# tk1363704/CAREL-VAE

Measured on AMD Instinct MI355X. Metric: clause-pairs/sec (training step), higher is better.
Workload: dtype bf16

## Files before the change

### carel_vae_amd/csrc/carel_hip_internal.h

```cpp
#pragma once
#include <hip/hip_runtime.h>
#include <stdarg.h>
#include <stdio.h>
#include "../../include/carel_hip.h"
#include "carel_common.h"

#ifdef CAREL_EXPERIMENTS
#define CAREL_TUNABLE(type, name, value) static type name = value
#else
#define CAREL_TUNABLE(type, name, value) static constexpr type name = value
#endif

namespace carel {

int set_error(int code, const char* fmt, ...);
int check_launch(const char* what);
int slab_reduce_multi(const void* slabs, void* out, int64_t n, const void* slabs2, void* out2, int64_t n2, int splits, const void* partials,
                      int nparts, void* dgamma, void* dbeta, void* dbias, hipStream_t stream);
#ifdef CAREL_EXPERIMENTS
int gemm_rowln_wanted(long rows);
int gemm_rowln_wanted_k(int K);
#else
inline int gemm_rowln_wanted(long) { return 0; }
inline int gemm_rowln_wanted_k(int) { return 0; }
#endif
void encoder_ln_resid_enable(int on);
void encoder_ln_slab_fusion_enable(int on);
void encoder_wgrad_group_enable(int on);
void adam_grid_cap(long cap);
void tail_overlap_enable(int on);
int gemm_pp_init_device(int device);
int gather_rows(const void* in_f32, const void* in_bf16, const void* idx, int n, void* out_f32, void* out_bf16, hipStream_t stream);
int scatter_rows(const void* in_f32, const void* in_bf16, const void* idx, int n, void* out_f32, void* out_bf16, hipStream_t stream);

int layernorm_bwd_rows(const void* dy, const void* h, const void* stats, const void* gamma, int64_t rows, uint32_t drop_seed, uint32_t drop_site,
                       uint32_t drop_idx_offset, float drop_p, const void* drop_row_map, void* dh_f32, void* dy_bf16, void* partials,
                       hipStream_t stream);
int layernorm_bwd_reduce(const void* partials, int64_t rows, void* dgamma, void* dbeta, void* dbias, hipStream_t stream);
int layernorm_bwd_blocks_max(int64_t rows);
int layernorm_bwd_rows_slabs(const void* slabs, int splits, const void* resid, const void* h, const void* stats, const void* gamma, int64_t rows,
                             uint32_t drop_seed, uint32_t drop_site, uint32_t drop_idx_offset, float drop_p, const void* drop_row_map, void* dh_f32,
                             void* dy_bf16, void* partials, hipStream_t stream);
int layernorm_fwd_slabs(const void* slabs, int splits, const void* bias, const void* resid, const void* resid_stats, const void* resid_gamma,
                        const void* resid_beta, uint32_t drop_seed, uint32_t drop_site, uint32_t drop_idx_offset, float drop_p, const void* drop_row_map,
                        void* h_out, const void* gamma, const void* beta, float eps, int64_t rows, void* x_f32, void* x_bf16, void* stats,
                        hipStream_t stream);

constexpr int GEMM_EX_FIXED_ROWS = 0x100;
constexpr int GEMM_EX_DEFER_EPILOGUE = 0x200;
int gemm_bf16_ex(const carel_gemm_args* a, int split_tile_factor, void* stream);
int gemm_bf16_split_plan(const carel_gemm_args* a, int split_tile_factor);
int gemm_wgrad_splits_max(int M, int N, long T);
int embed_ln_bwd_ex(const carel_embed_args* a, const void* dx0, void* dword, void* dpos, void* dtype_, void* dgamma, void* dbeta,
                    void* partials, void* row_scratch, hipStream_t stream, const void* sort_ws = nullptr);
int embed_sort_supported(const carel_embed_args* a);
size_t embed_sort_bytes();
int embed_ln_fwd_keys(const carel_embed_args* a, void* sort_ws, hipStream_t stream);
int embed_sort_rows(const carel_embed_args* a, void* sort_ws, hipStream_t stream);

struct WgradGroupProb { const void* dY; const void* X; void* dW; void* db; int M, N; };
struct WgradGroupLn { const void* partials; int nparts; void* dgamma; void* dbeta; void* dbias; };
size_t gemm_pp_wgrad_group_ws_bytes(const WgradGroupProb* pb, int n, long T);
int gemm_pp_wgrad_group_ok(const WgradGroupProb* pb, int n, long T);
int gemm_pp_wgrad_group(const WgradGroupProb* pb, int n, long T, void* ws, size_t ws_bytes, const WgradGroupLn* ln, int n_ln, hipStream_t stream);

inline Dropout make_dropout(uint32_t seed, uint32_t site, float p, uint32_t idx_offset) {
  Dropout d;
  d.key = mix32(seed + site * 0x9E3779B9u);
  d.idx_offset = idx_offset;
  if (p <= 0.f) { d.thresh = 0u; d.scale = 1.f; }
  else if (p >= 1.f) { d.thresh = 0xFFFFFFFFu; d.scale = 0.f; }
  else {
    d.thresh = (uint32_t)((double)p * 4294967296.0);
    d.scale = (float)(1.0 / (1.0 - (double)p));
    if (d.thresh == 0u) d.scale = 1.f;
  }
  return d;
}

struct AttnParams;
int attn_long_fwd(const AttnParams& q, hipStream_t stream);
int attn_long_bwd(const AttnParams& q, void* workspace, int64_t workspace_bytes, hipStream_t stream);

}
```

### carel_vae_amd/csrc/gemm.hip

```cpp
#include "gemm_epilogue.h"
#include "reduce_device.h"

namespace carel {

template <int EPI>
__global__ __launch_bounds__(256) void slab_epilogue_kernel(GemmParams p, const float* __restrict__ slabs, int splits) {
  const long chunk = (long)blockIdx.x * 256 + threadIdx.x;
  const int cpr = p.N >> 3;
  if (chunk >= (long)p.M * cpr) return;
  const long row = chunk / cpr, col = (chunk - row * cpr) * 8;
  const long off = row * p.N + col, plane = (long)p.M * p.N;
  float v[8];
  {
    const float4 a = *(const float4*)(slabs + off), b = *(const float4*)(slabs + off + 4);
    v[0] = a.x; v[1] = a.y; v[2] = a.z; v[3] = a.w; v[4] = b.x; v[5] = b.y; v[6] = b.z; v[7] = b.w;
  }
  for (int z = 1; z < splits; ++z) {
    const float4 a = *(const float4*)(slabs + z * plane + off), b = *(const float4*)(slabs + z * plane + off + 4);
    v[0] += a.x; v[1] += a.y; v[2] += a.z; v[3] += a.w; v[4] += b.x; v[5] += b.y; v[6] += b.z; v[7] += b.w;
  }
  epi_store8<EPI>(p, v, row, col);
}

template <bool AT, bool BT, int EPI, int DBG = 0>
// ... 672 lines not shown
    std::vector<float> c2;
    for (size_t i = 0; i + 1 < g_prof.cal2.size(); i += 2) {
      float t = 0.f;
      if (hipEventSynchronize(g_prof.cal2[i + 1]) == hipSuccess && hipEventElapsedTime(&t, g_prof.cal2[i], g_prof.cal2[i + 1]) == hipSuccess) c2.push_back(t);
    }
    if (!c2.empty()) { std::sort(c2.begin(), c2.end()); g_prof.last_pair_us = c2[c2.size() / 2] * 1e3; }
  }
  for (size_t i = 0; i + 1 < g_prof.used; i += 2) {
    if (hipEventSynchronize(g_prof.ev[i + 1]) != hipSuccess) return set_error(CAREL_ERR_HIP, "carel_profile_gemm_read: event sync failed");
    float t = 0.f;
    if (hipEventElapsedTime(&t, g_prof.ev[i], g_prof.ev[i + 1]) != hipSuccess) return set_error(CAREL_ERR_HIP, "carel_profile_gemm_read: elapsed failed");
    ms += (t > overhead ? t - overhead : 0.0); fl += g_prof.flops[i / 2];
  }
  *total_ms = ms; *total_flops = fl; *launches = (int64_t)(g_prof.used / 2);
  g_prof.used = 0; g_prof.flops.clear();
  return CAREL_OK;
}

extern "C" int carel_profile_gemm_overheads(double* empty_kernel_bracket_us, double* event_pair_us) {
  if (!empty_kernel_bracket_us || !event_pair_us) return set_error(CAREL_ERR_ARG, "carel_profile_gemm_overheads: null output");
  *empty_kernel_bracket_us = g_prof.last_empty_us; *event_pair_us = g_prof.last_pair_us;
  return CAREL_OK;
}

static int gemm_shape_ok(int M, int N, int K, int splits, int form) {
  if (M <= 0 || N <= 0 || K <= 0 || splits <= 0) return 0;
  if (form == CAREL_GEMM_TN) {
    if (M % 256 == 0 && N % 96 == 0 && K % 64 == 0 && (K >> 6) / splits >= 4) return 1;
  }
  const bool pp = form != CAREL_GEMM_TN && N % 96 == 0 && K >= 256;
  if (!((M % 128 == 0 && N % 128 == 0) || (M % 256 == 0 && N % 192 == 0) || pp)) return 0;
  if (K % (64 * splits)) return 0;
  return 1;
}

#ifdef CAREL_EXPERIMENTS
CAREL_TUNABLE(int, g_rowln_mode, 0);
CAREL_TUNABLE(long, g_rowln_min_rows, 6144);
namespace carel {
int gemm_rowln_wanted(long rows) { return g_rowln_mode != 0 && rows >= g_rowln_min_rows; }
int gemm_rowln_wanted_k(int K) { return g_rowln_mode == 1 || K <= 768; }
}
extern "C" int carel_gemm_rowln(const carel_gemm_rowln_args* a, void* stream_) {
  hipStream_t stream = (hipStream_t)stream_;
  if (!a) return set_error(CAREL_ERR_ARG, "carel_gemm_rowln: null args");
  if (a->M < 1 || a->K < 128 || (a->K & 127)) return set_error(CAREL_ERR_SHAPE, "carel_gemm_rowln: M >= 1 and K a multiple of 128 (M=%d K=%d)", a->M, a->K);
  if (!a->A || !a->W || !a->resid_f32 || !a->gamma || !a->beta) return set_error(CAREL_ERR_ARG, "carel_gemm_rowln: null operand");
  if ((((uintptr_t)a->A | (uintptr_t)a->W | (uintptr_t)a->resid_f32 | (uintptr_t)a->gamma | (uintptr_t)a->beta | (uintptr_t)a->bias | (uintptr_t)a->h_f32 |
        (uintptr_t)a->x_f32 | (uintptr_t)a->x_bf16) & 15) || (a->lda & 7) || a->lda < a->K || (!a->w_packed && ((a->ldb & 7) || a->ldb < a->K)))
    return set_error(CAREL_ERR_ARG, "carel_gemm_rowln: operands must be 16-byte aligned, leading dimensions multiples of 8 and >= K");
  RowLnParams p;
  p.A = (const bf16_t*)a->A; p.lda = a->lda; p.W = (const bf16_t*)a->W; p.ldb = a->ldb; p.bias = (const float*)a->bias; p.resid = (const float*)a->resid_f32;
  p.gamma = (const float*)a->gamma; p.beta = (const float*)a->beta; p.eps = a->eps;
  p.h_out = (float*)a->h_f32; p.x_f32 = (float*)a->x_f32; p.x_bf16 = (bf16_t*)a->x_bf16; p.stats = (float*)a->stats; p.M = a->M; p.K = a->K;
  p.drop = make_dropout(a->drop_seed, a->drop_site, a->drop_p, a->drop_idx_offset); p.drop_row_map = (const int*)a->drop_row_map;
  ProfScope prof_scope(stream, 2.0 * (double)a->M * 768.0 * (double)a->K);
  return gemm_rowln_launch(p, a->w_packed != 0, stream);
}
extern "C" int carel_gemm_rowln_pack(const void* W, int64_t ldb, int32_t K, void* out, void* stream) {
  if (!W || !out || K < 128 || (K & 127) || ldb < K || (ldb & 7) || (((uintptr_t)W | (uintptr_t)out) & 15))
    return set_error(CAREL_ERR_ARG, "carel_gemm_rowln_pack: bad arguments (K multiple of 128, ldb >= K multiple of 8, 16-byte aligned pointers)");
  return gemm_rowln_pack(W, (long)ldb, K, out, (hipStream_t)stream);
}

extern "C" int carel_gemm_set_variant(int32_t v) {
  if (v >= 20 && v <= 23) { g_xcd_n = 1 << (v - 20); return CAREL_OK; }
  if (v == 24) { g_xcd_n = 0; return CAREL_OK; }
  if (v == 30 || v == 31) { g_big_auto = v - 30; return CAREL_OK; }
  if (v >= 50 && v <= 59) { g_pp_min_tiles = (v - 50) * 32; return CAREL_OK; }
  if (v >= 340 && v <= 342) { g_sm_mode = v - 340; return CAREL_OK; }
  if (v >= 330 && v <= 333) { g_resid_split = v - 330; return CAREL_OK; }
  if (v >= 40 && v <= 49) { g_pp_min_tiles_k768 = (v - 40) * 32; return CAREL_OK; }
  if (v >= 70 && v <= 73) { gemm_pp_force_npn(v - 70); return CAREL_OK; }
  if (v >= 100 && v <= 116) { gemm_pp_wgrad_force(v - 100); return CAREL_OK; }
  if (v == 130 || v == 131) { g_auto_split_min_k = v == 130 ? 1536 : 768; return CAREL_OK; }
  if (v == 140 || v == 141) { g_pp_split = v - 140; return CAREL_OK; }
  if (v == 160 || v == 161) { gemm_pp_gelu_lut(v - 160); return CAREL_OK; }
  if (v >= 190 && v <= 192) { g_rowln_mode = v - 190; return CAREL_OK; }
  if (v >= 193 && v <= 195) { gemm_rowln_dbg(v - 193); return CAREL_OK; }
  if (v == 270 || v == 271) { encoder_ln_slab_fusion_enable(v - 270); return CAREL_OK; }
  if (v >= 250 && v <= 252) { gemm_pp_group_mode(v - 250); return CAREL_OK; }
  if (v == 240 || v == 241) { encoder_wgrad_group_enable(v - 240); return CAREL_OK; }
  if (v == 230 || v == 231) { encoder_ln_resid_enable(v - 230); return CAREL_OK; }
  if (v >= 220 && v <= 225) { gemm_tri_enable(v - 220); return CAREL_OK; }
  if (v >= 280 && v <= 292) { adam_grid_cap(32L << (v - 280)); return CAREL_OK; }
  if (v == 210 || v == 211) { tail_overlap_enable(v - 210); return CAREL_OK; }
  if (v == 200 || v == 201) { gemm_pp_pair_enable(v - 200); return CAREL_OK; }
  if (v == 170 || v == 171) { gemm_pp_epi_prefetch(v - 170); return CAREL_OK; }
  if (v == 120 || v == 121) { gemm_pp_xcd_rect(v - 120); return CAREL_OK; }
  if (v == 90 || v == 91) { gemm_pp_wide_variant(v - 90); return CAREL_OK; }
  g_gemm_variant = v;
  return CAREL_OK;
}
#endif

static int gemm_prepare(const carel_gemm_args* a, int split_tile_factor, PlannedGemm* out) {
  if (!a) return set_error(CAREL_ERR_ARG, "carel_gemm_bf16: null args");
  const int splits = a->splits > 0 ? a->splits : 1;
  if (!gemm_shape_ok(a->M, a->N, a->K, splits, a->form))
    return set_error(CAREL_ERR_SHAPE, "carel_gemm_bf16: (M,N) must be multiples of (128,128) or (256,192) and K of 64*splits (M=%d N=%d K=%d splits=%d)",
                     a->M, a->N, a->K, splits);
  if (!a->A || !a->B) return set_error(CAREL_ERR_ARG, "carel_gemm_bf16: null operand");
  if (((uintptr_t)a->A | (uintptr_t)a->B) & 15 || (a->lda & 7) || (a->ldb & 7) || (a->ldc & 3))
    return set_error(CAREL_ERR_ARG, "carel_gemm_bf16: operands must be 16-byte aligned, ld multiples of 8");
  GemmParams p = {};
  p.A = (const bf16_t*)a->A; p.B = (const bf16_t*)a->B; p.lda = a->lda; p.ldb = a->ldb;
  p.M = a->M; p.N = a->N; p.K = a->K / splits;
  p.out0 = (bf16_t*)a->out_bf16; p.out1 = (bf16_t*)a->out2_bf16; p.outf = (float*)a->out_f32; p.ldc = a->ldc;
  p.bias = (const float*)a->bias; p.resid = (const float*)a->resid_f32; p.aux = (const bf16_t*)a->aux_bf16;
  p.resid_stats = (const float*)a->resid_ln_stats; p.resid_gamma = (const float*)a->resid_ln_gamma; p.resid_beta = (const float*)a->resid_ln_beta;
  if (p.resid_stats || p.resid_gamma || p.resid_beta) {
    if (a->epilogue != EPI_BIAS_DROP_RESID || !p.resid_stats || !p.resid_gamma || !p.resid_beta)
      return set_error(CAREL_ERR_ARG, "carel_gemm_bf16: resid_ln_stats / _gamma / _beta go together and with CAREL_EPI_BIAS_DROP_RESID only");
    if ((((uintptr_t)p.resid_stats) & 7) || (((uintptr_t)p.resid_gamma | (uintptr_t)p.resid_beta) & 15))
      return set_error(CAREL_ERR_ARG, "carel_gemm_bf16: resid_ln_* pointers must be 8 / 16-byte aligned");
  }
  p.drop = make_dropout(a->drop_seed, a->drop_site, a->drop_p, a->drop_idx_offset);
  p.tiles_m = a->M / 128; p.tiles_n = a->N / 128;
  p.split_tile_factor = split_tile_factor;
  p.xcd_n = (a->form == CAREL_GEMM_TN && g_xcd_n <= 1) ? 8 : g_xcd_n;
  p.splitk_ws = (float*)a->splitk_ws; p.splitk_ws_bytes = a->splitk_ws ? (size_t)a->splitk_ws_bytes : 0;
  p.pair_flags = nullptr; p.pair_seq = 0;
  if (a->splitk_ws && a->splitk_ws_zeroed && (size_t)a->splitk_ws_bytes > (size_t)(64 << 20) && ((uintptr_t)a->splitk_ws & 15) == 0 && (a->splitk_ws_bytes & 15) == 0) {
    p.splitk_ws_bytes -= PP_PAIR_FLAG_BYTES;
    p.pair_flags = (unsigned*)((char*)a->splitk_ws + p.splitk_ws_bytes);
  }
  if (a->ldc != a->N) p.splitk_ws = nullptr;
  if (a->colsum_part) p.splitk_ws = nullptr;
  p.colsum_part = (float*)a->colsum_part; p.drop_row_map = (const int*)a->drop_row_map; p.colsum_a = (float*)a->colsum_a;
  if (p.colsum_a && a->form != CAREL_GEMM_TN) return set_error(CAREL_ERR_ARG, "carel_gemm_bf16: colsum_a is a TN-form (wgrad) option");
  const int form = a->form, epi = a->epilogue;
  if (splits != 1 && epi != EPI_SLAB_F32) return set_error(CAREL_ERR_ARG, "carel_gemm_bf16: split-K only with the slab epilogue");
#define NEED(ptr, what) if (!(ptr)) return set_error(CAREL_ERR_ARG, "carel_gemm_bf16: epilogue needs " what)
  switch (epi) {
    case EPI_BIAS_BF16: NEED(p.out0, "out_bf16"); break;
    case EPI_BIAS_GELU: NEED(p.out1, "out2_bf16"); break;
    case EPI_BIAS_GELU_DG: NEED(p.out0, "out_bf16"); NEED(p.out1, "out2_bf16"); break;
    case EPI_BIAS_DROP_RESID: NEED(p.outf, "out_f32"); NEED(p.resid, "resid_f32"); break;
    case EPI_DGELU_BF16: case EPI_MUL_BF16: NEED(p.out0, "out_bf16"); NEED(p.aux, "aux_bf16"); break;
    case EPI_ADD_F32: NEED(p.outf, "out_f32"); break;
    case EPI_SLAB_F32: NEED(p.outf, "out_f32"); break;
    default: return set_error(CAREL_ERR_ARG, "carel_gemm_bf16: unknown epilogue %d", epi);
  }
#undef NEED
  if (epi != EPI_BIAS_DROP_RESID && epi != EPI_ADD_F32 && epi != EPI_SLAB_F32 && (a->ldc & 7))
    return set_error(CAREL_ERR_ARG, "carel_gemm_bf16: bf16 outputs and aux need ldc a multiple of 8 (ldc=%ld)", (long)a->ldc);
  const auto fn = launch_instance(form, epi);
  if (!fn) return set_error(CAREL_ERR_ARG, "carel_gemm_bf16: unsupported form/epilogue combination (%d,%d)", form, epi);
  *out = PlannedGemm{p, splits, gemm_plan(p, form, epi, splits, a->K), fn};
  if (form == CAREL_GEMM_TN && out->plan.family == PLAN_PP) out->p.K = a->K;
  if (out->plan.family == PLAN_NONE)
    return set_error(CAREL_ERR_SHAPE, "carel_gemm_bf16: no kernel of this form takes the shape (M=%d N=%d K=%d splits=%d)", a->M, a->N, a->K, splits);
  return CAREL_OK;
}

extern "C" int carel_gemm_bf16(const carel_gemm_args* a, void* stream_) { return carel::gemm_bf16_ex(a, 1, stream_); }

int carel::gemm_bf16_split_plan(const carel_gemm_args* a, int split_tile_factor) {
  PlannedGemm g;
  return gemm_prepare(a, split_tile_factor, &g) ? 1 : g.plan.slabs;
}

#ifdef CAREL_EXPERIMENTS
extern "C" int carel_gemm_split_plan(const carel_gemm_args* a, int32_t flags, int32_t* plan) {
  if (!plan) return set_error(CAREL_ERR_ARG, "carel_gemm_split_plan: null plan");
  if (flags & ~(0xff | GEMM_EX_FIXED_ROWS)) return set_error(CAREL_ERR_ARG, "carel_gemm_split_plan: flags are a chain count | CAREL_PLAN_FIXED_ROWS");
// ... 97 lines not shown
```

### carel_vae_amd/csrc/ln.hip

```cpp
#include "carel_hip_internal.h"
#include "ln_device.h"
#include "reduce_device.h"

namespace carel {

__global__ __launch_bounds__(256) void ln_fwd_kernel(const float* __restrict__ h, const float* __restrict__ gamma,
                                                     const float* __restrict__ beta, float eps, long rows,
                                                     float* __restrict__ x_f32, bf16_t* __restrict__ x_bf16,
                                                     float* __restrict__ stats) {
  const int lane = threadIdx.x & 63;
  const long row = (long)blockIdx.x * 4 + (threadIdx.x >> 6);
  if (row >= rows) return;
  Row X = load_row(h + row * H, lane);
  const Row G = load_row(gamma, lane), Bt = load_row(beta, lane);
  float mean, rstd;
  ln_normalise(X, G, Bt, eps, mean, rstd);
  if (x_f32) store_row(x_f32 + row * H, lane, X);
  if (x_bf16) store_row_bf16(x_bf16 + row * H, lane, X);
  if (stats && lane == 0) { stats[row * 2] = mean; stats[row * 2 + 1] = rstd; }
}

struct LnFwdSlabs {
  const float* slabs; int splits; long plane;
  const float* bias; const float* resid; const float* resid_stats; const float* resid_gamma; const float* resid_beta;
// ... 35 lines not shown
  float mean, rstd;
  ln_normalise(X, G, Bt, eps, mean, rstd);
  if (x_f32) store_row(x_f32 + row * H, lane, X);
  if (x_bf16) store_row_bf16(x_bf16 + row * H, lane, X);
  if (stats && lane == 0) { stats[row * 2] = mean; stats[row * 2 + 1] = rstd; }
}

struct EmbedArgs {
  const long* ids; const long* tt;
  const float* word; const float* pos; const float* type;
  const float* gamma; const float* beta;
  float eps; int S; long rows; int roberta; int pad_id; int vocab, max_pos, type_vocab;
  Dropout drop;
  const int* tok_row;
};

__device__ __forceinline__ int position_id(const EmbedArgs& a, long row, int lane) {
  const int s = (int)(row % a.S);
  if (!a.roberta) return s;
  const long base = row - s;
  int cnt = 0;
  for (int c0 = 0; c0 <= s; c0 += 64) {
    const int j = c0 + lane;
    const bool nz = (j <= s) && (a.ids[base + j] != a.pad_id);
    cnt += __popcll(__ballot(nz));
  }
  const bool self_nz = a.ids[row] != a.pad_id;
  return (self_nz ? cnt : 0) + a.pad_id;
}

__device__ __forceinline__ Row embed_gather(const EmbedArgs& a, long row, int lane, int& pid, int& tid_) {
  long id = a.ids[row];
  id = id < 0 ? 0 : (id >= a.vocab ? a.vocab - 1 : id);
  pid = position_id(a, row, lane);
  pid = pid >= a.max_pos ? a.max_pos - 1 : pid;
  long t = a.tt ? a.tt[row] : 0;
  tid_ = (int)(t < 0 ? 0 : (t >= a.type_vocab ? a.type_vocab - 1 : t));
  Row A = load_row(a.word + id * H, lane);
  const Row B = load_row(a.pos + (long)pid * H, lane), Cc = load_row(a.type + (long)tid_ * H, lane);
  ROW_FOREACH(a = a + b + c; (void)e)
  return A;
}

__global__ __launch_bounds__(256) void embed_fwd_kernel(EmbedArgs a, float* __restrict__ x_f32, bf16_t* __restrict__ x_bf16,
                                                        float* __restrict__ stats, int2* __restrict__ row_keys) {
  const int lane = threadIdx.x & 63;
  const long orow = (long)blockIdx.x * 4 + (threadIdx.x >> 6);
  if (orow >= a.rows) return;
  const long row = a.tok_row ? (long)a.tok_row[orow] : orow;
  if (row_keys && lane == 0 && row < 0) row_keys[orow] = int2{-1, -1};
  if (row < 0) {
    Row Z;
#pragma unroll
    for (int i = 0; i < NV; ++i) Z.v[i] = float4{0.f, 0.f, 0.f, 0.f};
    store_row(x_f32 + orow * H, lane, Z);
    store_row_bf16(x_bf16 + orow * H, lane, Z);
    if (lane == 0) { stats[orow * 2] = 0.f; stats[orow * 2 + 1] = 0.f; }
    return;
  }
  int pid, tid_;
  Row X = embed_gather(a, row, lane, pid, tid_);
  if (row_keys && lane == 0) {
    long id = a.ids[row];
    id = id < 0 ? 0 : (id >= a.vocab ? a.vocab - 1 : id);
    row_keys[orow] = int2{(int)id, pid};
  }
  const Row G = load_row(a.gamma, lane), Bt = load_row(a.beta, lane);
  float mean, rstd;
  ln_normalise(X, G, Bt, a.eps, mean, rstd);
  if (a.drop.thresh) {
#pragma unroll
    for (int i = 0; i < NV; ++i) {
      const uint32_t e0 = (uint32_t)(row * H + (i * 64 + lane) * 4);
      float dm[4];
      dropout_mult_n<4>(a.drop, e0, dm);
      X.v[i].x *= dm[0]; X.v[i].y *= dm[1]; X.v[i].z *= dm[2]; X.v[i].w *= dm[3];
    }
  }
  store_row(x_f32 + orow * H, lane, X);
  store_row_bf16(x_bf16 + orow * H, lane, X);
  if (lane == 0) { stats[orow * 2] = mean; stats[orow * 2 + 1] = rstd; }
}

__device__ __forceinline__ void ln_bwd_row(Row& DY , Row& XH , const Row& G,
                                           float mean, float rstd) {
  float s1 = 0.f, s2 = 0.f;
#pragma unroll
  for (int i = 0; i < NV; ++i) {
    float* d = &DY.v[i].x; float* x = &XH.v[i].x; const float* g = &G.v[i].x;
#pragma unroll
    for (int e = 0; e < 4; ++e) {
      const float xh = (x[e] - mean) * rstd;
      const float dxh = d[e] * g[e];
      s1 += dxh; s2 += dxh * xh;
      x[e] = xh;
    }
  }
  s1 = wave_sum(s1) * (1.0f / H);
  s2 = wave_sum(s2) * (1.0f / H);
#pragma unroll
  for (int i = 0; i < NV; ++i) {
    float* d = &DY.v[i].x; float* x = &XH.v[i].x; const float* g = &G.v[i].x;
#pragma unroll
    for (int e = 0; e < 4; ++e) {
      const float dy = d[e], xh = x[e];
      d[e] = rstd * (dy * g[e] - s1 - xh * s2);
      x[e] = dy * xh;
    }
  }
}

constexpr int LNB_ROWS = 16;

__device__ __forceinline__ void write_partials(float* lds , const Row& acc, float* __restrict__ dst, int lane, int wave) {
  __syncthreads();
  store_row(lds + wave * H, lane, acc);
  __syncthreads();
  for (int c = threadIdx.x; c < H; c += 256) dst[c] = (lds[c] + lds[H + c]) + (lds[2 * H + c] + lds[3 * H + c]);
}

struct LnSlabSrc { int splits; long plane; const float* resid; };
template <bool SLAB, int RPW = 4>
__global__ __launch_bounds__(256) void ln_bwd_kernel(const float* __restrict__ dy_out, const float* __restrict__ h,
                                                     const float* __restrict__ stats, const float* __restrict__ gamma,
                                                     long rows, Dropout drop, const int* __restrict__ row_map,
                                                     float* __restrict__ dh, bf16_t* __restrict__ dyb,
                                                     float* __restrict__ partials, LnSlabSrc src) {
  __shared__ float lds[4 * H];
  const int lane = threadIdx.x & 63, wave = threadIdx.x >> 6;
  const Row G = load_row(gamma, lane);
  Row accG, accB, accBias;
#pragma unroll
  for (int i = 0; i < NV; ++i) accG.v[i] = accB.v[i] = accBias.v[i] = float4{0.f, 0.f, 0.f, 0.f};
  constexpr int WG_ROWS = 4 * RPW;
  Row DYr[RPW], XHr[RPW];
  float mr[RPW], rr[RPW];
  int dr[RPW];
  const int* rm = row_map ? row_map : (const int*)stats;
#pragma unroll
  for (int k = 0; k < RPW; ++k) {
    const long row = (long)blockIdx.x * WG_ROWS + wave + 4 * k;
    const long lrow = row < rows ? row : rows - 1;
    DYr[k] = load_row(dy_out + lrow * H, lane);
    if constexpr (SLAB) {
      for (int z = 1; z < src.splits; ++z) {
        const Row Z = load_row(dy_out + (long)z * src.plane + lrow * H, lane);
#pragma unroll
        for (int i = 0; i < NV; ++i) { DYr[k].v[i].x += Z.v[i].x; DYr[k].v[i].y += Z.v[i].y; DYr[k].v[i].z += Z.v[i].z; DYr[k].v[i].w += Z.v[i].w; }
      }
      if (src.resid) {
        const Row R = load_row(src.resid + lrow * H, lane);
#pragma unroll
        for (int i = 0; i < NV; ++i) { DYr[k].v[i].x += R.v[i].x; DYr[k].v[i].y += R.v[i].y; DYr[k].v[i].z += R.v[i].z; DYr[k].v[i].w += R.v[i].w; }
      }
    }
    XHr[k] = load_row(h + lrow * H, lane);
    mr[k] = stats[lrow * 2]; rr[k] = stats[lrow * 2 + 1];
    dr[k] = rm[lrow];
  }
#pragma unroll
  for (int k = 0; k < RPW; ++k) {
    const long row = (long)blockIdx.x * WG_ROWS + wave + 4 * k;
    if (row >= rows) break;
    Row DY = DYr[k];
    Row XH = XHr[k];
    const float mean = mr[k], rstd = rr[k];
#pragma unroll
    for (int i = 0; i < NV; ++i) { accB.v[i].x += DY.v[i].x; accB.v[i].y += DY.v[i].y; accB.v[i].z += DY.v[i].z; accB.v[i].w += DY.v[i].w; }
    ln_bwd_row(DY, XH, G, mean, rstd);
#pragma unroll
    for (int i = 0; i < NV; ++i) { accG.v[i].x += XH.v[i].x; accG.v[i].y += XH.v[i].y; accG.v[i].z += XH.v[i].z; accG.v[i].w += XH.v[i].w; }
    if (dh) store_row(dh + row * H, lane, DY);
    if (drop.thresh) {
      const long drow = row_map ? (long)dr[k] : row;
#pragma unroll
      for (int i = 0; i < NV; ++i) {
        const uint32_t e0 = (uint32_t)(drow * H + (i * 64 + lane) * 4);
        float dm[4];
        dropout_mult_n<4>(drop, e0, dm);
        DY.v[i].x *= dm[0]; DY.v[i].y *= dm[1]; DY.v[i].z *= dm[2]; DY.v[i].w *= dm[3];
      }
    }
    if (dyb) store_row_bf16(dyb + row * H, lane, DY);
#pragma unroll
    for (int i = 0; i < NV; ++i) { accBias.v[i].x += DY.v[i].x; accBias.v[i].y += DY.v[i].y; accBias.v[i].z += DY.v[i].z; accBias.v[i].w += DY.v[i].w; }
  }
  float* dst = partials + (long)blockIdx.x * 3 * H;
  write_partials(lds, accG, dst, lane, wave);
  write_partials(lds, accB, dst + H, lane, wave);
  write_partials(lds, accBias, dst + 2 * H, lane, wave);
}

__global__ __launch_bounds__(256) void pos_reduce_kernel(const float* __restrict__ rows, int B, int S, float* __restrict__ dpos) {
  const long e = ((long)blockIdx.x * 256 + threadIdx.x) * 4;
  if (e >= (long)S * H) return;
  float4 acc = float4{0.f, 0.f, 0.f, 0.f};
  for (int b = 0; b < B; b += 4) {
    float4 v[4];
#pragma unroll
    for (int u = 0; u < 4; ++u) v[u] = (b + u < B) ? *(const float4*)(rows + (long)(b + u) * S * H + e) : float4{0.f, 0.f, 0.f, 0.f};
#pragma unroll
    for (int u = 0; u < 4; ++u) { acc.x += v[u].x; acc.y += v[u].y; acc.z += v[u].z; acc.w += v[u].w; }
  }
  *(float4*)(dpos + e) = acc;
}

constexpr int EMB_SORT_MAX = 8192, EMB_ROW_BITS = 13;
__global__ __launch_bounds__(1024) void embed_sort_kernel(const int2* __restrict__ row_keys, int rows, uint32_t* __restrict__ out) {
  __shared__ uint32_t k[EMB_SORT_MAX];
  const int which = (int)blockIdx.x;
  int n = 64;
  while (n < rows) n <<= 1;
  for (int i = threadIdx.x; i < n; i += 1024) {
    uint32_t key = 0xFFFFFFFFu;
    if (i < rows) {
      const int2 v = row_keys[i];
      const int id = which ? v.y : v.x;
      if (id >= 0) key = ((uint32_t)id << EMB_ROW_BITS) | (uint32_t)i;
    }
    k[i] = key;
  }
  __syncthreads();
  for (int size = 2; size <= n; size <<= 1)
    for (int stride = size >> 1; stride > 0; stride >>= 1) {
      for (int t = threadIdx.x; t < (n >> 1); t += 1024) {
        const int lo = 2 * t - (t & (stride - 1)), hi = lo + stride;
        const bool up = (lo & size) == 0;
        const uint32_t a = k[lo], b = k[hi];
        if ((a > b) == up) { k[lo] = b; k[hi] = a; }
      }
      __syncthreads();
    }
  for (int i = threadIdx.x; i < EMB_SORT_MAX; i += 1024) out[which * EMB_SORT_MAX + i] = i < n ? k[i] : 0xFFFFFFFFu;
}

__global__ __launch_bounds__(256) void embed_segsum_kernel(const uint32_t* __restrict__ keys, const float* __restrict__ rows, float* __restrict__ table,
                                                           int table_rows) {
  const int lane = threadIdx.x & 63;
  const int w = (int)blockIdx.x * 4 + (int)(threadIdx.x >> 6);
  const int pos = w / 3, chunk = w - pos * 3;
  if (pos >= EMB_SORT_MAX) return;
  const uint32_t key = keys[pos];
  if (key == 0xFFFFFFFFu) return;
  const uint32_t id = key >> EMB_ROW_BITS;
  if ((int)id >= table_rows) return;
  if (pos > 0 && (keys[pos - 1] >> EMB_ROW_BITS) == id) return;
  const float* src = rows + chunk * 256 + lane * 4;
  float4 acc = float4{0.f, 0.f, 0.f, 0.f};
  for (int base = pos; base < EMB_SORT_MAX; base += 64) {
    const uint32_t kj = base + lane < EMB_SORT_MAX ? keys[base + lane] : 0xFFFFFFFFu;
    const unsigned long long m = __ballot(kj != 0xFFFFFFFFu && (kj >> EMB_ROW_BITS) == id);
    const int cnt = m == ~0ull ? 64 : __ffsll((long long)~m) - 1;
#pragma unroll 8
    for (int t = 0; t < cnt; ++t) {
      const uint32_t r = (uint32_t)__shfl((int)kj, t, 64) & (uint32_t)(EMB_SORT_MAX - 1);
      const float4 v = *(const float4*)(src + (long)r * H);
      acc.x += v.x; acc.y += v.y; acc.z += v.z; acc.w += v.w;
    }
    if (cnt < 64) break;
  }
  *(float4*)(table + (long)id * H + chunk * 256 + lane * 4) = acc;
}

__global__ __launch_bounds__(256) void embed_bwd_kernel(EmbedArgs a, const float* __restrict__ dx0,
                                                        const float* __restrict__ stats, float* __restrict__ dword,
                                                        float* __restrict__ dpos, float* __restrict__ partials,
                                                        float* __restrict__ row_out, int word_atomic, int pos_atomic) {
  __shared__ float lds[4 * H];
  const int lane = threadIdx.x & 63, wave = threadIdx.x >> 6;
  const Row G = load_row(a.gamma, lane);
  Row accG, accB, accT0, accT1;
#pragma unroll
  for (int i = 0; i < NV; ++i) accG.v[i] = accB.v[i] = accT0.v[i] = accT1.v[i] = float4{0.f, 0.f, 0.f, 0.f};
  for (int r = wave; r < LNB_ROWS; r += 4) {
// ... 205 lines not shown
}
int embed_sort_rows(const carel_embed_args* a, void* sort_ws, hipStream_t stream) {
  const long rows = (a->tok_row && a->n_rows > 0) ? (long)a->n_rows : (long)a->batch * a->seq_len;
  hipLaunchKernelGGL(embed_sort_kernel, dim3(2), dim3(1024), 0, stream, (const int2*)sort_ws, (int)rows, (uint32_t*)((char*)sort_ws + (size_t)EMB_SORT_MAX * 8));
  return check_launch("embed_sort_kernel");
}
}

extern "C" int carel_embed_ln_bwd_blocks(int64_t rows) { return (int)((rows + LNB_ROWS - 1) / LNB_ROWS); }

namespace carel {
int embed_ln_bwd_ex(const carel_embed_args* a, const void* dx0, void* dword, void* dpos, void* dtype_, void* dgamma, void* dbeta,
                    void* partials, void* row_scratch, hipStream_t stream, const void* sort_ws) {
  int rc = embed_check(a, "carel_embed_ln_bwd");
  if (rc) return rc;
  if (!dx0 || !dword || !dpos || !dtype_ || !dgamma || !dbeta || !partials || !a->stats)
    return set_error(CAREL_ERR_ARG, "carel_embed_ln_bwd: null tensor");
  EmbedArgs e = make_embed(a);
  const int nblk = carel_embed_ln_bwd_blocks(e.rows);
  const int slots = 2 + e.type_vocab;
  const bool by_reduction = row_scratch && !e.roberta && !e.tok_row && e.rows == (long)a->batch * a->seq_len;
  const bool sorted = row_scratch && sort_ws && embed_sort_supported(a);
  hipLaunchKernelGGL(embed_bwd_kernel, dim3(nblk), dim3(256), 0, stream, e, (const float*)dx0, (const float*)a->stats,
                     (float*)dword, (float*)dpos, (float*)partials, (by_reduction || sorted) ? (float*)row_scratch : (float*)nullptr,
                     sorted ? 0 : 1, (by_reduction || sorted) ? 0 : 1);
  rc = check_launch("embed_bwd_kernel");
  if (rc) return rc;
  if (by_reduction) {
    hipLaunchKernelGGL(pos_reduce_kernel, dim3((unsigned)(((long)a->seq_len * H / 4 + 255) / 256)), dim3(256), 0, stream,
                       (const float*)row_scratch, a->batch, a->seq_len, (float*)dpos);
    if ((rc = check_launch("pos_reduce_kernel"))) return rc;
  }
  if (sorted) {
    const uint32_t* keys = (const uint32_t*)((const char*)sort_ws + (size_t)EMB_SORT_MAX * 8);
    const unsigned blocks = (unsigned)((EMB_SORT_MAX * 3 + 3) / 4);
    hipLaunchKernelGGL(embed_segsum_kernel, dim3(blocks), dim3(256), 0, stream, keys, (const float*)row_scratch, (float*)dword, a->vocab_size);
    if ((rc = check_launch("embed_segsum_kernel"))) return rc;
    if (!by_reduction) {
      hipLaunchKernelGGL(embed_segsum_kernel, dim3(blocks), dim3(256), 0, stream, keys + EMB_SORT_MAX, (const float*)row_scratch, (float*)dpos, a->max_pos);
      if ((rc = check_launch("embed_segsum_kernel"))) return rc;
    }
  }
  SegOuts so; so.p[0] = (float*)dgamma; so.p[1] = (float*)dbeta; so.p[2] = (float*)dtype_;
  so.p[3] = e.type_vocab > 1 ? (float*)dtype_ + H : nullptr;
  hipLaunchKernelGGL(partial_reduce_seg_kernel, dim3((slots * H + PR_COLS - 1) / PR_COLS), dim3(256), 0, stream, (const float*)partials,
                     so, H, slots * H, nblk);
  return check_launch("partial_reduce_seg_kernel");
}
}

extern "C" int carel_embed_ln_bwd(const carel_embed_args* a, const void* dx0, void* dword, void* dpos, void* dtype_,
                                  void* dgamma, void* dbeta, void* partials, void* stream_) {
  return embed_ln_bwd_ex(a, dx0, dword, dpos, dtype_, dgamma, dbeta, partials, nullptr, (hipStream_t)stream_, nullptr);
}

extern "C" int carel_layernorm_fwd(const void* h, const void* gamma, const void* beta, float eps, int64_t rows, int32_t hidden,
                                   void* x_f32, void* x_bf16, void* stats, void* stream_) {
  hipStream_t stream = (hipStream_t)stream_;
  if (hidden != H) return set_error(CAREL_ERR_SHAPE, "carel_layernorm_fwd: hidden must be %d", H);
  if (!h || !gamma || !beta || rows <= 0) return set_error(CAREL_ERR_ARG, "carel_layernorm_fwd: bad arguments");
  hipLaunchKernelGGL(ln_fwd_kernel, dim3((unsigned)((rows + 3) / 4)), dim3(256), 0, stream, (const float*)h, (const float*)gamma,
                     (const float*)beta, eps, (long)rows, (float*)x_f32, (bf16_t*)x_bf16, (float*)stats);
  return check_launch("ln_fwd_kernel");
}

static int ln_bwd_rpw(int64_t rows) { return rows <= 2048 ? 1 : (rows <= 4096 ? 2 : 4); }
extern "C" int carel_layernorm_bwd_blocks(int64_t rows) { const int wg = 4 * ln_bwd_rpw(rows); return (int)((rows + wg - 1) / wg); }
namespace carel {
int layernorm_bwd_blocks_max(int64_t rows) {
  if (rows <= 2048) return (int)((rows + 3) / 4);
  const int64_t big = (rows + 15) / 16;
  return (int)(big > 512 ? big : 512);
}
}

extern "C" int carel_layernorm_bwd(const void* dy, const void* h, const void* stats, const void* gamma, int64_t rows,
                                   int32_t hidden, uint32_t drop_seed, uint32_t drop_site, uint32_t drop_idx_offset,
                                   float drop_p, void* dh_f32, void* dy_bf16, void* dgamma, void* dbeta, void* dbias,
                                   void* partials, void* stream_) {
  return carel_layernorm_bwd_packed(dy, h, stats, gamma, rows, hidden, drop_seed, drop_site, drop_idx_offset, drop_p, nullptr, dh_f32,
                                    dy_bf16, dgamma, dbeta, dbias, partials, stream_);
}

namespace carel {
int layernorm_bwd_rows(const void* dy, const void* h, const void* stats, const void* gamma, int64_t rows, uint32_t drop_seed, uint32_t drop_site,
                       uint32_t drop_idx_offset, float drop_p, const void* drop_row_map, void* dh_f32, void* dy_bf16, void* partials,
                       hipStream_t stream) {
  if (!dy || !h || !stats || !gamma || !partials || rows <= 0) return set_error(CAREL_ERR_ARG, "carel_layernorm_bwd: bad arguments");
  const int nblk = carel_layernorm_bwd_blocks(rows);
  const Dropout drop = make_dropout(drop_seed, drop_site, drop_p, drop_idx_offset);
  const LnSlabSrc src{1, 0, nullptr};
#define CAREL_LNB(R) hipLaunchKernelGGL((ln_bwd_kernel<false, R>), dim3(nblk), dim3(256), 0, stream, (const float*)dy, (const float*)h, (const float*)stats, \
                     (const float*)gamma, (long)rows, drop, (const int*)drop_row_map, (float*)dh_f32, (bf16_t*)dy_bf16, (float*)partials, src)
  switch (ln_bwd_rpw(rows)) { case 1: CAREL_LNB(1); break; case 2: CAREL_LNB(2); break; default: CAREL_LNB(4); }
#undef CAREL_LNB
  return check_launch("ln_bwd_kernel");
}
int layernorm_bwd_rows_slabs(const void* slabs, int splits, const void* resid, const void* h, const void* stats, const void* gamma, int64_t rows,
                             uint32_t drop_seed, uint32_t drop_site, uint32_t drop_idx_offset, float drop_p, const void* drop_row_map, void* dh_f32,
                             void* dy_bf16, void* partials, hipStream_t stream) {
  if (!slabs || splits < 2 || !h || !stats || !gamma || !partials || rows <= 0) return set_error(CAREL_ERR_ARG, "layernorm_bwd_rows_slabs: bad arguments");
  const int nblk = carel_layernorm_bwd_blocks(rows);
  const Dropout drop = make_dropout(drop_seed, drop_site, drop_p, drop_idx_offset);
  const LnSlabSrc src{splits, (long)rows * H, (const float*)resid};
#define CAREL_LNB(R) hipLaunchKernelGGL((ln_bwd_kernel<true, R>), dim3(nblk), dim3(256), 0, stream, (const float*)slabs, (const float*)h, (const float*)stats, \
                     (const float*)gamma, (long)rows, drop, (const int*)drop_row_map, (float*)dh_f32, (bf16_t*)dy_bf16, (float*)partials, src)
  switch (ln_bwd_rpw(rows)) { case 1: CAREL_LNB(1); break; case 2: CAREL_LNB(2); break; default: CAREL_LNB(4); }
#undef CAREL_LNB
  return check_launch("ln_bwd_kernel<slabs>");
}
int layernorm_fwd_slabs(const void* slabs, int splits, const void* bias, const void* resid, const void* resid_stats, const void* resid_gamma,
                        const void* resid_beta, uint32_t drop_seed, uint32_t drop_site, uint32_t drop_idx_offset, float drop_p, const void* drop_row_map,
                        void* h_out, const void* gamma, const void* beta, float eps, int64_t rows, void* x_f32, void* x_bf16, void* stats,
                        hipStream_t stream) {
  if (!slabs || splits < 2 || !resid || !gamma || !beta || rows <= 0) return set_error(CAREL_ERR_ARG, "layernorm_fwd_slabs: bad arguments");
  if (resid_stats && (!resid_gamma || !resid_beta)) return set_error(CAREL_ERR_ARG, "layernorm_fwd_slabs: recomputed residual needs gamma and beta");
  LnFwdSlabs a;
  a.slabs = (const float*)slabs; a.splits = splits; a.plane = (long)rows * H; a.bias = (const float*)bias; a.resid = (const float*)resid;
  a.resid_stats = (const float*)resid_stats; a.resid_gamma = (const float*)resid_gamma; a.resid_beta = (const float*)resid_beta;
  a.drop = make_dropout(drop_seed, drop_site, drop_p, drop_idx_offset); a.row_map = (const int*)drop_row_map; a.h_out = (float*)h_out;
  hipLaunchKernelGGL(ln_fwd_slabs_kernel, dim3((unsigned)((rows + 3) / 4)), dim3(256), 0, stream, a, (const float*)gamma, (const float*)beta, eps, (long)rows,
                     (float*)x_f32, (bf16_t*)x_bf16, (float*)stats);
  return check_launch("ln_fwd_slabs_kernel");
}
int layernorm_bwd_reduce(const void* partials, int64_t rows, void* dgamma, void* dbeta, void* dbias, hipStream_t stream) {
  const int nblk = carel_layernorm_bwd_blocks(rows);
  SegOuts so; so.p[0] = (float*)dgamma; so.p[1] = (float*)dbeta; so.p[2] = (float*)dbias; so.p[3] = nullptr;
  hipLaunchKernelGGL(partial_reduce_seg_kernel, dim3((3 * H + PR_COLS - 1) / PR_COLS), dim3(256), 0, stream, (const float*)partials, so,
                     H, 3 * H, nblk);
  return check_launch("partial_reduce_seg_kernel");
}
}

extern "C" int carel_layernorm_bwd_packed(const void* dy, const void* h, const void* stats, const void* gamma, int64_t rows,
                                          int32_t hidden, uint32_t drop_seed, uint32_t drop_site, uint32_t drop_idx_offset,
                                          float drop_p, const void* drop_row_map, void* dh_f32, void* dy_bf16, void* dgamma,
                                          void* dbeta, void* dbias, void* partials, void* stream_) {
  hipStream_t stream = (hipStream_t)stream_;
  if (hidden != H) return set_error(CAREL_ERR_SHAPE, "carel_layernorm_bwd: hidden must be %d", H);
  int rc = layernorm_bwd_rows(dy, h, stats, gamma, rows, drop_seed, drop_site, drop_idx_offset, drop_p, drop_row_map, dh_f32, dy_bf16,
                              partials, stream);
  if (rc) return rc;
  return layernorm_bwd_reduce(partials, rows, dgamma, dbeta, dbias, stream);
}

extern "C" int carel_colsum_bf16(const void* x, int64_t ld, int64_t rows, int32_t n, void* out_f32, int32_t accumulate,
                                 void* partials, void* stream_) {
  hipStream_t stream = (hipStream_t)stream_;
  if (!x || !out_f32 || !partials || rows <= 0 || n <= 0 || (n & 7) || (ld & 7))
    return set_error(CAREL_ERR_ARG, "carel_colsum_bf16: bad arguments (n, ld multiples of 8)");
  const int chunks = (int)((rows + 255) / 256);
  hipLaunchKernelGGL(colsum_bf16_kernel, dim3((n + 255) / 256, chunks), dim3(256), 0, stream, (const bf16_t*)x, (long)ld,
                     (long)rows, n, (float*)partials);
  int rc = check_launch("colsum_bf16_kernel");
  if (rc) return rc;
  hipLaunchKernelGGL(partial_reduce_kernel, dim3((n + PR_COLS - 1) / PR_COLS), dim3(256), 0, stream, (const float*)partials, (float*)out_f32, n,
                     chunks, accumulate);
  return check_launch("partial_reduce_kernel");
}

extern "C" int carel_partial_reduce_f32(const void* partials, void* out, int32_t n, int32_t nparts, int32_t accumulate, void* stream_) {
  hipStream_t stream = (hipStream_t)stream_;
  if (!partials || !out || n <= 0 || nparts <= 0) return set_error(CAREL_ERR_ARG, "carel_partial_reduce_f32: bad arguments");
  hipLaunchKernelGGL(partial_reduce_kernel, dim3((n + PR_COLS - 1) / PR_COLS), dim3(256), 0, stream, (const float*)partials, (float*)out, n, nparts, accumulate);
  return check_launch("partial_reduce_kernel");
}
```

Baseline: 8423.

## Software-pipeline LayerNorm backward rows with capped VGPRs for higher occupancy

Replaces the RPW=4 LayerNorm backward kernel with a paired form. It loads one row ahead instead of holding all four rows in registers, and pins VGPRs and waves-per-EU to 4 waves. It also keeps gamma in LDS, uses a DPP/swizzle wave reduction, shrinks LDS to two rows, and uses a staged tree reduction for the partials. The aim is to raise occupancy and overlap memory latency with compute in the LN backward pass, at the cost of more barriers and possible register spills.

New measurement: 8413. No clear change (-0.1%).

```diff
diff --git a/carel_vae_amd/csrc/carel_hip_internal.h b/carel_vae_amd/csrc/carel_hip_internal.h
--- a/carel_vae_amd/csrc/carel_hip_internal.h
+++ b/carel_vae_amd/csrc/carel_hip_internal.h
@@ -27,6 +27,7 @@
 void encoder_ln_resid_enable(int on);
 void encoder_ln_slab_fusion_enable(int on);
 void encoder_wgrad_group_enable(int on);
+void ln_bwd_paired_enable(int on);
 void adam_grid_cap(long cap);
 void tail_overlap_enable(int on);
 int gemm_pp_init_device(int device);
diff --git a/carel_vae_amd/csrc/gemm.hip b/carel_vae_amd/csrc/gemm.hip
--- a/carel_vae_amd/csrc/gemm.hip
+++ b/carel_vae_amd/csrc/gemm.hip
@@ -778,6 +778,7 @@
   if (v >= 250 && v <= 252) { gemm_pp_group_mode(v - 250); return CAREL_OK; }
   if (v == 240 || v == 241) { encoder_wgrad_group_enable(v - 240); return CAREL_OK; }
   if (v == 230 || v == 231) { encoder_ln_resid_enable(v - 230); return CAREL_OK; }
+  if (v == 350 || v == 351) { ln_bwd_paired_enable(v - 350); return CAREL_OK; }
   if (v >= 220 && v <= 225) { gemm_tri_enable(v - 220); return CAREL_OK; }
   if (v >= 280 && v <= 292) { adam_grid_cap(32L << (v - 280)); return CAREL_OK; }
   if (v == 210 || v == 211) { tail_overlap_enable(v - 210); return CAREL_OK; }
diff --git a/carel_vae_amd/csrc/ln.hip b/carel_vae_amd/csrc/ln.hip
--- a/carel_vae_amd/csrc/ln.hip
+++ b/carel_vae_amd/csrc/ln.hip
@@ -141,6 +141,16 @@
   if (lane == 0) { stats[orow * 2] = mean; stats[orow * 2 + 1] = rstd; }
 }
 
+__device__ __forceinline__ float wave_sum_swz(float v) {
+  v += __int_as_float(__builtin_amdgcn_ds_bpermute((int)(((threadIdx.x & 63) ^ 32) << 2), __float_as_int(v)));
+  v += __int_as_float(__builtin_amdgcn_ds_swizzle(__float_as_int(v), (16 << 10) | 0x1f));
+  v += __int_as_float(__builtin_amdgcn_ds_swizzle(__float_as_int(v), (8 << 10) | 0x1f));
+  v += __int_as_float(__builtin_amdgcn_ds_swizzle(__float_as_int(v), (4 << 10) | 0x1f));
+  v += __int_as_float(__builtin_amdgcn_ds_swizzle(__float_as_int(v), (2 << 10) | 0x1f));
+  v += __int_as_float(__builtin_amdgcn_ds_swizzle(__float_as_int(v), (1 << 10) | 0x1f));
+  return v;
+}
+template <bool SWZ = false>
 __device__ __forceinline__ void ln_bwd_row(Row& DY , Row& XH , const Row& G,
                                            float mean, float rstd) {
   float s1 = 0.f, s2 = 0.f;
@@ -155,8 +165,8 @@
       x[e] = xh;
     }
   }
-  s1 = wave_sum(s1) * (1.0f / H);
-  s2 = wave_sum(s2) * (1.0f / H);
+  s1 = (SWZ ? wave_sum_swz(s1) : wave_sum(s1)) * (1.0f / H);
+  s2 = (SWZ ? wave_sum_swz(s2) : wave_sum(s2)) * (1.0f / H);
 #pragma unroll
   for (int i = 0; i < NV; ++i) {
     float* d = &DY.v[i].x; float* x = &XH.v[i].x; const float* g = &G.v[i].x;
@@ -178,14 +188,67 @@
   for (int c = threadIdx.x; c < H; c += 256) dst[c] = (lds[c] + lds[H + c]) + (lds[2 * H + c] + lds[3 * H + c]);
 }
 
+__device__ __forceinline__ void write_partials_staged(float* lds , const Row& acc, float* __restrict__ dst, int lane, int wave) {
+  __syncthreads();
+  if (wave & 1) store_row(lds + (wave >> 1) * H, lane, acc);
+  __syncthreads();
+  Row s = acc;
+  if (!(wave & 1)) {
+    const Row o = load_row(lds + (wave >> 1) * H, lane);
+#pragma unroll
+    for (int i = 0; i < NV; ++i) { s.v[i].x += o.v[i].x; s.v[i].y += o.v[i].y; s.v[i].z += o.v[i].z; s.v[i].w += o.v[i].w; }
+  }
+  __syncthreads();
+  if (wave == 2) store_row(lds + H, lane, s);
+  __syncthreads();
+  if (wave == 0) {
+    const Row o = load_row(lds + H, lane);
+#pragma unroll
+    for (int i = 0; i < NV; ++i) { s.v[i].x += o.v[i].x; s.v[i].y += o.v[i].y; s.v[i].z += o.v[i].z; s.v[i].w += o.v[i].w; }
+    store_row(dst, lane, s);
+  }
+}
+
 struct LnSlabSrc { int splits; long plane; const float* resid; };
-template <bool SLAB, int RPW = 4>
-__global__ __launch_bounds__(256) void ln_bwd_kernel(const float* __restrict__ dy_out, const float* __restrict__ h,
-                                                     const float* __restrict__ stats, const float* __restrict__ gamma,
-                                                     long rows, Dropout drop, const int* __restrict__ row_map,
-                                                     float* __restrict__ dh, bf16_t* __restrict__ dyb,
-                                                     float* __restrict__ partials, LnSlabSrc src) {
-  __shared__ float lds[4 * H];
+template <bool SLAB>
+__device__ __forceinline__ Row ln_bwd_load_dy(const float* __restrict__ dy_out, long lrow, int lane, const LnSlabSrc& src) {
+  Row D = load_row(dy_out + lrow * H, lane);
+  if constexpr (SLAB) {
+    for (int z = 1; z < src.splits; ++z) {
+      const Row Z = load_row(dy_out + (long)z * src.plane + lrow * H, lane);
+#pragma unroll
+      for (int i = 0; i < NV; ++i) { D.v[i].x += Z.v[i].x; D.v[i].y += Z.v[i].y; D.v[i].z += Z.v[i].z; D.v[i].w += Z.v[i].w; }
+    }
+    if (src.resid) {
+      const Row R = load_row(src.resid + lrow * H, lane);
+#pragma unroll
+      for (int i = 0; i < NV; ++i) { D.v[i].x += R.v[i].x; D.v[i].y += R.v[i].y; D.v[i].z += R.v[i].z; D.v[i].w += R.v[i].w; }
+    }
+  }
+  return D;
+}
+__device__ __forceinline__ void ln_bwd_store(Row& DY, long row, long drow, int lane, const Dropout& drop, float* __restrict__ dh,
+                                             bf16_t* __restrict__ dyb, Row& accBias) {
+  if (dh) store_row(dh + row * H, lane, DY);
+  if (drop.thresh) {
+#pragma unroll
+    for (int i = 0; i < NV; ++i) {
+      const uint32_t e0 = (uint32_t)(drow * H + (i * 64 + lane) * 4);
+      float dm[4];
+      dropout_mult_n<4>(drop, e0, dm);
+      DY.v[i].x *= dm[0]; DY.v[i].y *= dm[1]; DY.v[i].z *= dm[2]; DY.v[i].w *= dm[3];
+    }
+  }
+  if (dyb) store_row_bf16(dyb + row * H, lane, DY);
+#pragma unroll
+  for (int i = 0; i < NV; ++i) { accBias.v[i].x += DY.v[i].x; accBias.v[i].y += DY.v[i].y; accBias.v[i].z += DY.v[i].z; accBias.v[i].w += DY.v[i].w; }
+}
+
+template <bool SLAB, int RPW>
+__device__ __forceinline__ void ln_bwd_upfront(float* lds , const float* __restrict__ dy_out, const float* __restrict__ h,
+                                               const float* __restrict__ stats, const float* __restrict__ gamma, long rows, const Dropout& drop,
+                                               const int* __restrict__ row_map, float* __restrict__ dh, bf16_t* __restrict__ dyb,
+                                               float* __restrict__ partials, const LnSlabSrc& src) {
   const int lane = threadIdx.x & 63, wave = threadIdx.x >> 6;
   const Row G = load_row(gamma, lane);
   Row accG, accB, accBias;
@@ -200,19 +263,7 @@
   for (int k = 0; k < RPW; ++k) {
     const long row = (long)blockIdx.x * WG_ROWS + wave + 4 * k;
     const long lrow = row < rows ? row : rows - 1;
-    DYr[k] = load_row(dy_out + lrow * H, lane);
-    if constexpr (SLAB) {
-      for (int z = 1; z < src.splits; ++z) {
-        const Row Z = load_row(dy_out + (long)z * src.plane + lrow * H, lane);
-#pragma unroll
-        for (int i = 0; i < NV; ++i) { DYr[k].v[i].x += Z.v[i].x; DYr[k].v[i].y += Z.v[i].y; DYr[k].v[i].z += Z.v[i].z; DYr[k].v[i].w += Z.v[i].w; }
-      }
-      if (src.resid) {
-        const Row R = load_row(src.resid + lrow * H, lane);
-#pragma unroll
-        for (int i = 0; i < NV; ++i) { DYr[k].v[i].x += R.v[i].x; DYr[k].v[i].y += R.v[i].y; DYr[k].v[i].z += R.v[i].z; DYr[k].v[i].w += R.v[i].w; }
-      }
-    }
+    DYr[k] = ln_bwd_load_dy<SLAB>(dy_out, lrow, lane, src);
     XHr[k] = load_row(h + lrow * H, lane);
     mr[k] = stats[lrow * 2]; rr[k] = stats[lrow * 2 + 1];
     dr[k] = rm[lrow];
@@ -229,26 +280,102 @@
     ln_bwd_row(DY, XH, G, mean, rstd);
 #pragma unroll
     for (int i = 0; i < NV; ++i) { accG.v[i].x += XH.v[i].x; accG.v[i].y += XH.v[i].y; accG.v[i].z += XH.v[i].z; accG.v[i].w += XH.v[i].w; }
-    if (dh) store_row(dh + row * H, lane, DY);
-    if (drop.thresh) {
-      const long drow = row_map ? (long)dr[k] : row;
-#pragma unroll
-      for (int i = 0; i < NV; ++i) {
-        const uint32_t e0 = (uint32_t)(drow * H + (i * 64 + lane) * 4);
-        float dm[4];
-        dropout_mult_n<4>(drop, e0, dm);
-        DY.v[i].x *= dm[0]; DY.v[i].y *= dm[1]; DY.v[i].z *= dm[2]; DY.v[i].w *= dm[3];
-      }
-    }
-    if (dyb) store_row_bf16(dyb + row * H, lane, DY);
-#pragma unroll
-    for (int i = 0; i < NV; ++i) { accBias.v[i].x += DY.v[i].x; accBias.v[i].y += DY.v[i].y; accBias.v[i].z += DY.v[i].z; accBias.v[i].w += DY.v[i].w; }
+    ln_bwd_store(DY, row, row_map ? (long)dr[k] : row, lane, drop, dh, dyb, accBias);
   }
   float* dst = partials + (long)blockIdx.x * 3 * H;
   write_partials(lds, accG, dst, lane, wave);
   write_partials(lds, accB, dst + H, lane, wave);
   write_partials(lds, accBias, dst + 2 * H, lane, wave);
 }
+
+constexpr int LNB4_VGPRS = 112, LNB4_LDS_ROWS = 2;
+template <class T>
+__device__ __forceinline__ long ln_row_after(long row, T after) {
+  asm volatile("" : "+s"(row) : "v"(after));
+  const unsigned lo = __builtin_amdgcn_readfirstlane((unsigned)row), hi = __builtin_amdgcn_readfirstlane((unsigned)((unsigned long)row >> 32));
+  return (long)(((unsigned long)hi << 32) | lo);
+}
+template <bool SLAB, bool EARLY, bool GREG0>
+__device__ __forceinline__ void ln_bwd_paired(float* lds , const float* __restrict__ dy_out, const float* __restrict__ h,
+                                              const float* __restrict__ stats, const float* __restrict__ gamma, long rows, const Dropout& drop,
+                                              const int* __restrict__ row_map, float* __restrict__ dh, bf16_t* __restrict__ dyb,
+                                              float* __restrict__ partials, const LnSlabSrc& src) {
+  constexpr int RPW = 4, WG_ROWS = 4 * RPW;
+  const int lane = threadIdx.x & 63, wave = __builtin_amdgcn_readfirstlane(threadIdx.x >> 6);
+  Row accG, accB, accBias;
+#pragma unroll
+  for (int i = 0; i < NV; ++i) accG.v[i] = accB.v[i] = accBias.v[i] = float4{0.f, 0.f, 0.f, 0.f};
+  const int* rm = row_map ? row_map : (const int*)stats;
+  const long row0 = (long)blockIdx.x * WG_ROWS + wave;
+  Row DYn, XHn;
+  float mn, rn;
+  int dn;
+#define CAREL_LNB_REQUEST(k, after) { \
+    long lrow_ = row0 + 4 * (k) < rows ? row0 + 4 * (k) : rows - 1; \
+    lrow_ = ln_row_after(lrow_, after); \
+    DYn = ln_bwd_load_dy<SLAB>(dy_out, lrow_, lane, src); \
+    XHn = load_row(h + lrow_ * H, lane); \
+    mn = stats[lrow_ * 2]; rn = stats[lrow_ * 2 + 1]; \
+    dn = rm[lrow_]; }
+  CAREL_LNB_REQUEST(0, lane)
+  const Row G0 = load_row(gamma, lane);
+#pragma unroll
+  for (int k = 0; k < RPW; ++k) {
+    const long row = row0 + 4 * k;
+    if (k == (GREG0 ? 1 : 0)) {
+      if (wave == 0) store_row(lds, lane, G0);
+      __syncthreads();
+    }
+    if (row >= rows) { if (k == 0) continue; else break; }
+    Row DY = DYn;
+    Row XH = XHn;
+    const float mean = mn, rstd = rn;
+    const long drow = row_map ? (long)dn : row;
+#pragma unroll
+    for (int i = 0; i < NV; ++i) { accB.v[i].x += DY.v[i].x; accB.v[i].y += DY.v[i].y; accB.v[i].z += DY.v[i].z; accB.v[i].w += DY.v[i].w; }
+    if (GREG0 && k == 0) {
+      ln_bwd_row<true>(DY, XH, G0, mean, rstd);
+    } else {
+      const Row G = load_row(lds, lane);
+      ln_bwd_row<true>(DY, XH, G, mean, rstd);
+    }
+#pragma unroll
+    for (int i = 0; i < NV; ++i) { accG.v[i].x += XH.v[i].x; accG.v[i].y += XH.v[i].y; accG.v[i].z += XH.v[i].z; accG.v[i].w += XH.v[i].w; }
+    if (EARLY && k + 1 < RPW) CAREL_LNB_REQUEST(k + 1, accG.v[NV - 1].w)
+    ln_bwd_store(DY, ln_row_after(row, lane), drow, lane, drop, dh, dyb, accBias);
+    if (!EARLY && k + 1 < RPW) CAREL_LNB_REQUEST(k + 1, accBias.v[NV - 1].w)
+  }
+#undef CAREL_LNB_REQUEST
+  float* dst = partials + (long)blockIdx.x * 3 * H;
+  write_partials_staged(lds, accG, dst, lane, wave);
+  write_partials_staged(lds, accB, dst + H, lane, wave);
+  write_partials_staged(lds, accBias, dst + 2 * H, lane, wave);
+}
+
+#define CAREL_LNB_PARAMS const float* __restrict__ dy_out, const float* __restrict__ h, const float* __restrict__ stats, const float* __restrict__ gamma, \
+                         long rows, Dropout drop, const int* __restrict__ row_map, float* __restrict__ dh, bf16_t* __restrict__ dyb,                    \
+                         float* __restrict__ partials, LnSlabSrc src
+template <bool SLAB, int RPW = 4>
+__global__ __launch_bounds__(256) void ln_bwd_kernel(CAREL_LNB_PARAMS) {
+  static_assert(RPW < 4, "the dense form is specialised below");
+  __shared__ float lds[4 * H];
+  ln_bwd_upfront<SLAB, RPW>(lds, dy_out, h, stats, gamma, rows, drop, row_map, dh, dyb, partials, src);
+}
+template <> __global__ __launch_bounds__(256) __attribute__((amdgpu_waves_per_eu(4, 4), amdgpu_num_vgpr(LNB4_VGPRS / 2))) void ln_bwd_kernel<false, 4>(CAREL_LNB_PARAMS) {
+  __shared__ float lds[LNB4_LDS_ROWS * H];
+  ln_bwd_paired<false, true, true>(lds, dy_out, h, stats, gamma, rows, drop, row_map, dh, dyb, partials, src);
+}
+template <> __global__ __launch_bounds__(256) __attribute__((amdgpu_waves_per_eu(4, 4), amdgpu_num_vgpr(LNB4_VGPRS / 2))) void ln_bwd_kernel<true, 4>(CAREL_LNB_PARAMS) {
+  __shared__ float lds[LNB4_LDS_ROWS * H];
+  ln_bwd_paired<true, false, false>(lds, dy_out, h, stats, gamma, rows, drop, row_map, dh, dyb, partials, src);
+}
+#ifdef CAREL_EXPERIMENTS
+template <bool SLAB>
+__global__ __launch_bounds__(256) void ln_bwd_upfront4_kernel(CAREL_LNB_PARAMS) {
+  __shared__ float lds[4 * H];
+  ln_bwd_upfront<SLAB, 4>(lds, dy_out, h, stats, gamma, rows, drop, row_map, dh, dyb, partials, src);
+}
+#endif
 
 __global__ __launch_bounds__(256) void pos_reduce_kernel(const float* __restrict__ rows, int B, int S, float* __restrict__ dpos) {
   const long e = ((long)blockIdx.x * 256 + threadIdx.x) * 4;
@@ -620,6 +747,16 @@
                                     dy_bf16, dgamma, dbeta, dbias, partials, stream_);
 }
 
+CAREL_TUNABLE(int, g_ln_bwd_paired, 1);
+#ifdef CAREL_EXPERIMENTS
+namespace carel { void ln_bwd_paired_enable(int on) { g_ln_bwd_paired = on ? 1 : 0; } }
+#define CAREL_LNB4_KERNEL(S) (g_ln_bwd_paired ? ln_bwd_kernel<S, 4> : ln_bwd_upfront4_kernel<S>)
+#else
+#define CAREL_LNB4_KERNEL(S) (ln_bwd_kernel<S, 4>)
+#endif
+#define CAREL_LNB4(S, DYP) hipLaunchKernelGGL(CAREL_LNB4_KERNEL(S), dim3(nblk), dim3(256), 0, stream, (const float*)DYP, (const float*)h, (const float*)stats, \
+                     (const float*)gamma, (long)rows, drop, (const int*)drop_row_map, (float*)dh_f32, (bf16_t*)dy_bf16, (float*)partials, src)
+
 namespace carel {
 int layernorm_bwd_rows(const void* dy, const void* h, const void* stats, const void* gamma, int64_t rows, uint32_t drop_seed, uint32_t drop_site,
                        uint32_t drop_idx_offset, float drop_p, const void* drop_row_map, void* dh_f32, void* dy_bf16, void* partials,
@@ -630,7 +767,7 @@
   const LnSlabSrc src{1, 0, nullptr};
 #define CAREL_LNB(R) hipLaunchKernelGGL((ln_bwd_kernel<false, R>), dim3(nblk), dim3(256), 0, stream, (const float*)dy, (const float*)h, (const float*)stats, \
                      (const float*)gamma, (long)rows, drop, (const int*)drop_row_map, (float*)dh_f32, (bf16_t*)dy_bf16, (float*)partials, src)
-  switch (ln_bwd_rpw(rows)) { case 1: CAREL_LNB(1); break; case 2: CAREL_LNB(2); break; default: CAREL_LNB(4); }
+  switch (ln_bwd_rpw(rows)) { case 1: CAREL_LNB(1); break; case 2: CAREL_LNB(2); break; default: CAREL_LNB4(false, dy); }
 #undef CAREL_LNB
   return check_launch("ln_bwd_kernel");
 }
@@ -643,7 +780,7 @@
   const LnSlabSrc src{splits, (long)rows * H, (const float*)resid};
 #define CAREL_LNB(R) hipLaunchKernelGGL((ln_bwd_kernel<true, R>), dim3(nblk), dim3(256), 0, stream, (const float*)slabs, (const float*)h, (const float*)stats, \
                      (const float*)gamma, (long)rows, drop, (const int*)drop_row_map, (float*)dh_f32, (bf16_t*)dy_bf16, (float*)partials, src)
-  switch (ln_bwd_rpw(rows)) { case 1: CAREL_LNB(1); break; case 2: CAREL_LNB(2); break; default: CAREL_LNB(4); }
+  switch (ln_bwd_rpw(rows)) { case 1: CAREL_LNB(1); break; case 2: CAREL_LNB(2); break; default: CAREL_LNB4(true, slabs); }
 #undef CAREL_LNB
   return check_launch("ln_bwd_kernel<slabs>");
 }
```
